# hungdinhxuan/real-time-deepfake-speech-detection

Hardware: AMD Instinct MI355X
Metric: utterances/sec (4 s @ 16 kHz) (higher is better)
Workload: dtype fp16

## Files before the change

### real-time-deepfake-speech-detection_amd/csrc/afx_conformer.hip

```cpp
#include "afx_common.h"
#include "afx_kernels.h"

namespace afx {

__global__ void conf_tokens_kernel(const float* __restrict__ ll, const float* __restrict__ cls, float bn_scale,
                                   float bn_shift, int T, int E, float* __restrict__ out, int raw) {
  const int b = blockIdx.y;
  const long n = (long)(T + 1) * E;
  for (long i = (long)blockIdx.x * blockDim.x + threadIdx.x; i < n; i += (long)gridDim.x * blockDim.x) {
    const int row = (int)(i / E), c = (int)(i % E);
    float v;
    if (row == 0)
      v = cls[c];
    else if (raw)
      v = ll[((long)b * T + row - 1) * E + c];
    else
      v = selu(fmaf(ll[((long)b * T + row - 1) * E + c], bn_scale, bn_shift));
    out[(long)b * n + i] = v;
  }
}
const char* launch_conf_tokens(const float* ll, const float* cls, float bn_scale, float bn_shift, int B, int T,
                               int E, float* out, hipStream_t s, bool raw) {
  hipLaunchKernelGGL(conf_tokens_kernel, dim3(16, B), dim3(256), 0, s, ll, cls, bn_scale, bn_shift, T, E, out, raw ? 1 : 0);
  hipError_t e = hipGetLastError();
// ... 129 lines not shown
  if ((ldq % 4) || (ldkv % 4) || (ldo % 4)) return "conf_attn: row strides must be multiples of 4";
  hipError_t e = hipSuccess;
#define AFX_CA(DHv)                                                                                             \
  AFX_DISPATCH_HT(dtype, e = launch_conf_attn_t<DHv, HT, true>(q, ldq, kv, ldkv, rel, max_pos, B, N, H, out_h, ldo, s, lens, len_add))
  if (!rel) {
    if (dh != 64 || dtype != DT_FP32) return "conf_attn: the no-relative-term form is the fp32 trunk attention (dh 64)";
    e = launch_conf_attn_t<64, F32T, false>(q, ldq, kv, ldkv, nullptr, 0, B, N, H, out_h, ldo, s, lens, len_add);
  }
  else if (dh == 36) { AFX_CA(36); }
  else if (dh == 32) { AFX_CA(32); }
  else if (dh == 64) { AFX_CA(64); }
  else return "conf_attn: supported head dims are 32, 36 (emb 144 / 4 heads) and 64";
#undef AFX_CA
  return e == hipSuccess ? nullptr : hipGetErrorString(e);
}

constexpr int CA_KEYS = 224, CA_VT_STRIDE = 232, CA_RS = 228, CA_NKT = 14, CA_KS = 7;

template <class HT, int DH, int NW>
__global__ __launch_bounds__(64 * NW) void conf_attn_mfma_kernel(const float* __restrict__ q, long ldq,
                                                             const float* __restrict__ kv, long ldkv,
                                                             const typename HT::T* __restrict__ rel_h, int max_pos,
                                                             int N, int H, typename HT::T* __restrict__ out, long ldo,
                                                             const int* __restrict__ lens, int len_add) {
  typedef typename HT::T Tt;
  typedef typename HT::V8 V8;
  typedef typename HT::V4 V4;
  const int Nrow = N;
  if (lens) N = lens[blockIdx.y] + len_add;
  constexpr int DT = (DH + 15) / 16;
  static_assert(DH % 4 == 0 && DH <= 64, "head dim");
  extern __shared__ __attribute__((aligned(16))) float sm_f[];
  char* sm = (char*)sm_f;
  char* k_lds = sm;
  Tt* vt_lds = (Tt*)(sm + CA_KEYS * 128);
  float* r_lds = (float*)(sm + CA_KEYS * 128 + 16 * DT * CA_VT_STRIDE * 2);
  constexpr int NT = 64 * NW;

  const int h = blockIdx.x, b = blockIdx.y;
  const int tid = threadIdx.x, lane = tid & 63, wave = tid >> 6;
  const int inner = H * DH;
  for (int i = tid; i < (CA_KEYS * 128 + 16 * DT * CA_VT_STRIDE * 2) / 16; i += NT) ((u32x4*)sm)[i] = u32x4{0u, 0u, 0u, 0u};
  __syncthreads();
  {
    constexpr int IT = (209 * (DH / 4) + NT - 1) / NT;
    f32x4 kreg[IT], vreg[IT];
#pragma unroll
// ... 6 lines not shown
        vreg[it] = *(const f32x4*)(row + inner);
      }
    }
#pragma unroll
    for (int it = 0; it < IT; ++it) {
      const int idx = tid + it * NT;
      if (idx < N * (DH / 4)) {
        const int key = idx / (DH / 4), q4 = idx % (DH / 4);
        V4 kh;
#pragma unroll
        for (int i = 0; i < 4; ++i) kh[i] = (Tt)kreg[it][i];
        const int c = q4 >> 1;
        *(V4*)(k_lds + key * 128 + ((c ^ ((key >> 1) & 7)) * 16) + (q4 & 1) * 8) = kh;
#pragma unroll
        for (int i = 0; i < 4; ++i) vt_lds[(q4 * 4 + i) * CA_VT_STRIDE + key] = (Tt)vreg[it][i];
      }
    }
  }
  __syncthreads();

  const int ql = lane & 15, g = lane >> 4;
  const float scale = 1.0f / sqrtf((float)DH);
  float* rw = r_lds + wave * 16 * CA_RS;
  const int nqt = (N + 15) >> 4;
  for (int qt = wave; qt < nqt; qt += NW) {
    const int q0 = qt * 16;
    int qrow = q0 + ql;
    qrow = qrow < N ? qrow : N - 1;
    V8 qf[2];
    {
      const float* qp = q + ((long)b * Nrow + qrow) * ldq + h * DH;
#pragma unroll
      for (int ks = 0; ks < 2; ++ks)
#pragma unroll
        for (int half = 0; half < 2; ++half) {
          const int d = ks * 32 + g * 8 + half * 4;
          f32x4 t = f32x4{0.f, 0.f, 0.f, 0.f};
          if (d < DH) t = *(const f32x4*)(qp + d);
#pragma unroll
          for (int i = 0; i < 4; ++i) qf[ks][half * 4 + i] = (Tt)(t[i] * scale);
        }
    }
    auto read_e = [&](int rp, V8 (&ef)[2][2]) {
#pragma unroll
      for (int u = 0; u < 2; ++u) {
        int er = q0 + (rp + u) * 16 + ql - (N - 1);
        er = er < -max_pos ? -max_pos : (er > max_pos ? max_pos : er);
// ... 102 lines not shown
#pragma unroll
      for (int nt = 0; nt < DT; ++nt) o[nt] = HT::mfma(vf[nt], pf, o[nt]);
      __builtin_amdgcn_sched_barrier(0);
    }
    const int qi = q0 + ql;
    if (qi < N) {
#pragma unroll
      for (int nt = 0; nt < DT; ++nt) {
        const int d = nt * 16 + g * 4;
        if (d < DH) {
          V4 hv;
#pragma unroll
          for (int c = 0; c < 4; ++c) hv[c] = (Tt)(o[nt][c] * rinv);
          *(V4*)(out + ((long)b * Nrow + qi) * ldo + h * DH + d) = hv;
        }
      }
    }
  }
}

template <int DH, int NW>
__global__ __launch_bounds__(64 * NW) void conf_attn_split_kernel(const float* __restrict__ q, long ldq, const float* __restrict__ kv, long ldkv,
                                                                  const float* __restrict__ rel64, int max_pos, int N, int H,
                                                                  float* __restrict__ out, long ldo, const int* __restrict__ lens, int len_add) {
  typedef _Float16 Tt;
  typedef f16x8 V8;
  typedef f16x4 V4;
  const int Nrow = N;
  if (lens) N = lens[blockIdx.y] + len_add;
  constexpr int DT = (DH + 15) / 16;
  static_assert(DH % 4 == 0 && DH <= 64, "head dim");
  extern __shared__ __attribute__((aligned(16))) float sm_f[];
  char* sm = (char*)sm_f;
  constexpr int KB = CA_KEYS * 128, VB = 16 * DT * CA_VT_STRIDE * 2;
  char* k_lds[2] = {sm, sm + KB};
  Tt* vt_lds[2] = {(Tt*)(sm + 2 * KB), (Tt*)(sm + 2 * KB + VB)};
  float* r_lds = (float*)(sm + 2 * KB + 2 * VB);
  constexpr int NT = 64 * NW;
  const int h = blockIdx.x, b = blockIdx.y;
  const int tid = threadIdx.x, lane = tid & 63, wave = tid >> 6;
  const int inner = H * DH;
  auto split4 = [](const f32x4& a, V4& hi, V4& lo) {
#pragma unroll
    for (int i = 0; i < 4; ++i) {
      hi[i] = (Tt)a[i];
      lo[i] = (Tt)(a[i] - (float)hi[i]);
    }
// ... 27 lines not shown
      const int idx = tid + it * NT;
      if (idx < N * (DH / 4)) {
        const int key = idx / (DH / 4), q4 = idx % (DH / 4);
        V4 kh, kl, vh, vl;
        split4(kreg[it], kh, kl);
        split4(vreg[it], vh, vl);
        const int c = q4 >> 1;
        const int off = key * 128 + ((c ^ ((key >> 1) & 7)) * 16) + (q4 & 1) * 8;
        *(V4*)(k_lds[0] + off) = kh;
        *(V4*)(k_lds[1] + off) = kl;
#pragma unroll
        for (int i = 0; i < 4; ++i) {
          vt_lds[0][(q4 * 4 + i) * CA_VT_STRIDE + key] = vh[i];
          vt_lds[1][(q4 * 4 + i) * CA_VT_STRIDE + key] = vl[i];
        }
      }
    }
  }
  __syncthreads();

  const int ql = lane & 15, g = lane >> 4;
  const float scale = 1.0f / sqrtf((float)DH);
  float* rw = r_lds + wave * 16 * CA_RS;
  const int nqt = (N + 15) >> 4;
  for (int qt = wave; qt < nqt; qt += NW) {
    const int q0 = qt * 16;
    int qrow = q0 + ql;
    qrow = qrow < N ? qrow : N - 1;
    V8 qh[2], qlo[2];
    {
      const float* qp = q + ((long)b * Nrow + qrow) * ldq + h * DH;
#pragma unroll
      for (int ks = 0; ks < 2; ++ks) {
        f32x4 t[2];
#pragma unroll
        for (int half = 0; half < 2; ++half) {
          const int d = ks * 32 + g * 8 + half * 4;
          t[half] = f32x4{0.f, 0.f, 0.f, 0.f};
          if (d < DH) t[half] = *(const f32x4*)(qp + d);
        }
        split8(t[0], t[1], qh[ks], qlo[ks]);
      }
    }
    auto read_e = [&](int rp, f32x4 (&ef)[2][2][2]) {
#pragma unroll
      for (int u = 0; u < 2; ++u) {
        int er = q0 + (rp + u) * 16 + ql - (N - 1);
// ... 113 lines not shown
        o[nt] = FP16::mfma(vf[nt][1], ph, o[nt]);
        o[nt] = FP16::mfma(vf[nt][0], pl, o[nt]);
        o[nt] = FP16::mfma(vf[nt][0], ph, o[nt]);
      }
      __builtin_amdgcn_sched_barrier(0);
    }
    const int qi = q0 + ql;
    if (qi < N) {
#pragma unroll
      for (int nt = 0; nt < DT; ++nt) {
        const int d = nt * 16 + g * 4;
        if (d < DH) *(f32x4*)(out + ((long)b * Nrow + qi) * ldo + h * DH + d) = o[nt] * rinv;
      }
#ifdef SHAW_DBG
      if (g == 0) {
        out[((long)b * Nrow + qi) * ldo + h * DH + 0] = mx;
        out[((long)b * Nrow + qi) * ldo + h * DH + 1] = sum;
      }
#endif
    }
  }
}
const char* launch_conf_attn_split(const float* q, long ldq, const float* kv, long ldkv, const float* rel64, int max_pos, int B, int N,
                                   int H, int dh, float* out, long ldo, hipStream_t s, const int* lens, int len_add) {
  if (dh != 36) return "conf_attn_split: built for head dim 36 (emb 144 / 4 heads)";
  if (N <= 0 || N + 15 > CA_KEYS || B <= 0 || B > 65535) return "conf_attn_split: 1..209 tokens";
  if ((ldq % 4) || (ldkv % 4) || (ldo % 4)) return "conf_attn_split: row strides must be multiples of 4";
  constexpr int DT = 3, NW = 4;
  const int lds = 2 * CA_KEYS * 128 + 2 * 16 * DT * CA_VT_STRIDE * 2 + NW * 16 * CA_RS * 4;
  static LdsLimit lim;
  hipError_t e = lim.ensure((const void*)conf_attn_split_kernel<36, NW>, lds);
  if (e == hipSuccess) {
    hipLaunchKernelGGL((conf_attn_split_kernel<36, NW>), dim3(H, B), dim3(64 * NW), lds, s, q, ldq, kv, ldkv, rel64, max_pos, N, H, out, ldo, lens, len_add);
    e = hipGetLastError();
  }
  return e == hipSuccess ? nullptr : hipGetErrorString(e);
}

constexpr int CAL_KB = 128, CAL_VT_STRIDE = 136, CAL_RS = 148, CAL_NKT = 8, CAL_KS = 4, CAL_RT = 9;

template <class HT, int DH>
__global__ __launch_bounds__(256, 2) void conf_attn_mfma_long_kernel(const float* __restrict__ q, long ldq,
                                                                  const float* __restrict__ kv, long ldkv,
                                                                  const typename HT::T* __restrict__ rel_h, int max_pos,
                                                                  int N, int H, typename HT::T* __restrict__ out, long ldo,
                                                                  const int* __restrict__ lens, int len_add) {
  typedef typename HT::T Tt;
  typedef typename HT::V8 V8;
  typedef typename HT::V4 V4;
  const int Nrow = N;
  if (lens) N = lens[blockIdx.y] + len_add;
  constexpr int DT = (DH + 15) / 16;
  static_assert(DH % 4 == 0 && DH <= 64, "head dim");
  extern __shared__ __attribute__((aligned(16))) float sm_f[];
  char* sm = (char*)sm_f;
  char* k_lds = sm;
  Tt* vt_lds = (Tt*)(sm + CAL_KB * 128);
  float* r_lds = (float*)(sm + CAL_KB * 128 + 16 * DT * CAL_VT_STRIDE * 2);
  const int h = blockIdx.x, b = blockIdx.y;
  const int tid = threadIdx.x, lane = tid & 63, wave = tid >> 6;
  const int inner = H * DH;
  const int ql = lane & 15, g = lane >> 4;
  const int q0 = blockIdx.z * 64 + wave * 16;
  const float scale = 1.0f / sqrtf((float)DH);
  float* rw = r_lds + wave * 16 * CAL_RS;
  for (int i = tid; i < (CAL_KB * 128 + 16 * DT * CAL_VT_STRIDE * 2) / 16; i += 256) ((u32x4*)sm)[i] = u32x4{0u, 0u, 0u, 0u};
  V8 qf[2];
  {
    const int qrow = q0 + ql < N ? q0 + ql : N - 1;
// ... 26 lines not shown
        if (idx < nk * (DH / 4)) {
          const int key = idx / (DH / 4), q4 = idx % (DH / 4);
          const float* row = kv + ((long)b * Nrow + j0 + key) * ldkv + h * DH + q4 * 4;
          kreg[it] = *(const f32x4*)row;
          vreg[it] = *(const f32x4*)(row + inner);
        }
      }
#pragma unroll
      for (int it = 0; it < IT; ++it) {
        const int idx = tid + it * 256;
        if (idx < nk * (DH / 4)) {
          const int key = idx / (DH / 4), q4 = idx % (DH / 4);
          V4 kh;
#pragma unroll
          for (int i = 0; i < 4; ++i) kh[i] = (Tt)kreg[it][i];
          const int c = q4 >> 1;
          *(V4*)(k_lds + key * 128 + ((c ^ ((key >> 1) & 7)) * 16) + (q4 & 1) * 8) = kh;
#pragma unroll
          for (int i = 0; i < 4; ++i) vt_lds[(q4 * 4 + i) * CAL_VT_STRIDE + key] = (Tt)vreg[it][i];
        }
      }
    }
    __syncthreads();
    if (q0 >= N) continue;

    const int base = q0 - j0 - (CAL_KB - 1);
#pragma unroll
    for (int rp = 0; rp < CAL_RT; ++rp) {
      int er = base + rp * 16 + ql;
      er = er < -max_pos ? -max_pos : (er > max_pos ? max_pos : er);
      const Tt* ep = rel_h + (long)(er + max_pos) * 64 + g * 8;
      const V8 e0 = *(const V8*)ep, e1 = *(const V8*)(ep + 32);
      f32x4 r2 = f32x4{0.f, 0.f, 0.f, 0.f};
      r2 = HT::mfma(e0, qf[0], r2);
      r2 = HT::mfma(e1, qf[1], r2);
      *(f32x4*)(rw + ql * CAL_RS + rp * 16 + g * 4) = r2;
    }
    f32x4 s[CAL_NKT];
#pragma unroll
    for (int kp = 0; kp < CAL_NKT; kp += 2) {
      V8 kf[2][2];
#pragma unroll
      for (int u = 0; u < 2; ++u) {
        const int krow = (kp + u) * 16 + ql;
        const int sw = (krow >> 1) & 7;
#pragma unroll
        for (int ks = 0; ks < 2; ++ks) kf[u][ks] = *(const V8*)(k_lds + krow * 128 + (((ks * 4 + g) ^ sw) * 16));
// ... 35 lines not shown
      V8 pf;
#pragma unroll
      for (int c = 0; c < 4; ++c) {
        pf[c] = (Tt)s[2 * s2][c];
        pf[4 + c] = (Tt)s[2 * s2 + 1][c];
      }
      V8 vf[DT];
#pragma unroll
      for (int nt = 0; nt < DT; ++nt) {
        const Tt* vr = vt_lds + (nt * 16 + ql) * CAL_VT_STRIDE + s2 * 32 + g * 4;
        const V4 lo = *(const V4*)vr;
        const V4 hi = *(const V4*)(vr + 16);
#pragma unroll
        for (int c = 0; c < 4; ++c) {
          vf[nt][c] = lo[c];
          vf[nt][4 + c] = hi[c];
        }
      }
#pragma unroll
      for (int nt = 0; nt < DT; ++nt) o[nt] = HT::mfma(vf[nt], pf, o[nt]);
    }
  }
  const int qi = q0 + ql;
  if (qi < N) {
    const float rinv = 1.0f / l;
#pragma unroll
    for (int nt = 0; nt < DT; ++nt) {
      const int d = nt * 16 + g * 4;
      if (d < DH) {
        V4 hv;
#pragma unroll
        for (int c = 0; c < 4; ++c) hv[c] = (Tt)(o[nt][c] * rinv);
        *(V4*)(out + ((long)b * Nrow + qi) * ldo + h * DH + d) = hv;
      }
    }
  }
}

static int g_conf_attn_force_long = 0;
void conf_attn_mfma_set_force_long(int v) { g_conf_attn_force_long = v != 0; }
static int g_conf_attn_waves = 7;
void conf_attn_mfma_set_waves(int v) { g_conf_attn_waves = v == 4 ? 4 : 7; }

const char* launch_conf_attn_mfma(const float* q, long ldq, const float* kv, long ldkv, const void* rel_h, int max_pos,
                                  int B, int N, int H, int dh, void* out_h, long ldo, int dtype, hipStream_t s,
                                  const int* lens, int len_add) {
  if (dh != 36) return "conf_attn_mfma: built for head dim 36 (emb 144 / 4 heads)";
  if (N <= 0 || B <= 0 || B > 65535) return "conf_attn_mfma: bad shape";
  if (dtype == DT_FP32) return "conf_attn_mfma: half-precision operands only";
  if ((ldq % 4) || (ldkv % 4) || (ldo % 4)) return "conf_attn_mfma: row strides must be multiples of 4";
  constexpr int DT = 3;
  if (N + 15 > CA_KEYS || g_conf_attn_force_long) {
    const int ldsl = CAL_KB * 128 + 16 * DT * CAL_VT_STRIDE * 2 + 4 * 16 * CAL_RS * 4;
    hipError_t el = hipSuccess;
    static LdsLimit liml[2];
    dim3 grid(H, B, (N + 63) / 64);
    if (dtype == DT_BF16) {
      el = liml[0].ensure((const void*)conf_attn_mfma_long_kernel<BF16, 36>, ldsl);
      if (el == hipSuccess)
        hipLaunchKernelGGL((conf_attn_mfma_long_kernel<BF16, 36>), grid, dim3(256), ldsl, s, q, ldq, kv, ldkv, (const __bf16*)rel_h,
                           max_pos, N, H, (__bf16*)out_h, ldo, lens, len_add);
    } else {
      el = liml[1].ensure((const void*)conf_attn_mfma_long_kernel<FP16, 36>, ldsl);
      if (el == hipSuccess)
        hipLaunchKernelGGL((conf_attn_mfma_long_kernel<FP16, 36>), grid, dim3(256), ldsl, s, q, ldq, kv, ldkv, (const _Float16*)rel_h,
                           max_pos, N, H, (_Float16*)out_h, ldo, lens, len_add);
    }
    if (el == hipSuccess) el = hipGetLastError();
    return el == hipSuccess ? nullptr : hipGetErrorString(el);
  }
  const int nw = N > 64 && g_conf_attn_waves != 4 ? 7 : 4;
  const int lds = CA_KEYS * 128 + 16 * DT * CA_VT_STRIDE * 2 + nw * 16 * CA_RS * 4;
  hipError_t e = hipSuccess;
  static LdsLimit lim[4];
#define AFX_CAM(HTv, NWv, slot, Tv)                                                                                      \
  do {                                                                                                                   \
    e = lim[slot].ensure((const void*)conf_attn_mfma_kernel<HTv, 36, NWv>, lds);                                         \
    if (e == hipSuccess)                                                                                                 \
      hipLaunchKernelGGL((conf_attn_mfma_kernel<HTv, 36, NWv>), dim3(H, B), dim3(64 * NWv), lds, s, q, ldq, kv, ldkv,    \
                         (const Tv*)rel_h, max_pos, N, H, (Tv*)out_h, ldo, lens, len_add);                               \
  } while (0)
  if (dtype == DT_BF16) {
    if (nw == 7) AFX_CAM(BF16, 7, 0, __bf16); else AFX_CAM(BF16, 4, 1, __bf16);
  } else {
    if (nw == 7) AFX_CAM(FP16, 7, 2, _Float16); else AFX_CAM(FP16, 4, 3, _Float16);
  }
#undef AFX_CAM
  if (e == hipSuccess) e = hipGetLastError();
  return e == hipSuccess ? nullptr : hipGetErrorString(e);
}

template <class HT>
__global__ __launch_bounds__(256) void conf_dwconv_kernel(const float* __restrict__ x, long ldx,
                                                          const float* __restrict__ w, const float* __restrict__ bias,
                                                          const float* __restrict__ bn_scale,
                                                          const float* __restrict__ bn_shift, int N, int NC, int C, int k,
                                                          typename HT::T* __restrict__ out, long ldo,
                                                          const int* __restrict__ lens, int len_add) {
  typedef typename HT::T Tt;
  const int Nrow = N;
  if (lens) N = lens[blockIdx.y] + len_add;
  constexpr bool EXACT = sizeof(Tt) == 4;
  constexpr int KMAX = 31, TB = 8;
  extern __shared__ __attribute__((aligned(16))) float sm_f[];
  float* sm = sm_f;
  const int c0 = blockIdx.x * 32, b = blockIdx.y, tid = threadIdx.x;
  const int pl = k / 2;
  const int f0 = blockIdx.z * NC, nc = min(NC, N - f0);
  const int rows = nc + KMAX - 1 + TB;
  float* us = sm;
  const int cl = tid & 31, tl = tid >> 5;
  const int c = c0 + cl;
  const bool cok = c < C;
  for (int r = tl; r < rows; r += 8) {
    const int t = f0 + r - pl;
    float u = 0.f;
    if (cok && t >= 0 && t < N) {
      const float* row = x + ((long)b * Nrow + t) * ldx;
      u = row[c] * (EXACT ? sigmoid_acc(row[C + c]) : sigmoid_fast(row[C + c]));
    }
    us[r * 32 + cl] = u;
  }
  float wr[KMAX];
#pragma unroll
  for (int j = 0; j < KMAX; ++j) wr[j] = (cok && j < k) ? w[(long)c * k + j] : 0.f;
  const float bi = cok ? bias[c] : 0.f, sc = cok ? bn_scale[c] : 0.f, sh = cok ? bn_shift[c] : 0.f;
  __syncthreads();
  const int per = (nc + 7) / 8;
  const int t_end = min(nc, (tl + 1) * per);
  for (int t0 = tl * per; t0 < t_end; t0 += TB) {
    float win[TB + KMAX - 1];
#pragma unroll
    for (int i = 0; i < TB + KMAX - 1; ++i) win[i] = us[(t0 + i) * 32 + cl];
    float acc[TB];
#pragma unroll
    for (int u = 0; u < TB; ++u) acc[u] = bi;
#pragma unroll
    for (int j = 0; j < KMAX; ++j)
#pragma unroll
      for (int u = 0; u < TB; ++u) acc[u] = fmaf(wr[j], win[u + j], acc[u]);
    if (cok) {
#pragma unroll
      for (int u = 0; u < TB; ++u) {
        const float y = fmaf(acc[u], sc, sh);
        if (t0 + u < t_end) out[((long)b * Nrow + f0 + t0 + u) * ldo + c] = (Tt)(EXACT ? swish(y) : swish_fast(y));
      }
    }
  }
}

const char* launch_conf_dwconv(const float* x, long ldx, const float* w, const float* bias, const float* bn_scale,
                               const float* bn_shift, int B, int N, int C, int k, void* out_h, long ldo, int dtype,
                               hipStream_t s, const int* lens, int len_add) {
  if (k > 31) return "conf_dwconv: depthwise kernels up to 31 taps";
  if (N <= 0 || B <= 0 || B > 65535) return "conf_dwconv: bad shape";
  const int NC = N < 1024 ? N : 1024;
  const int lds = (NC + 31 - 1 + 8) * 32 * (int)sizeof(float);
  dim3 grid((C + 31) / 32, B, (N + NC - 1) / NC);
  hipError_t e = hipSuccess;
  static LdsLimit lim[3];
  if (dtype < 0 || dtype > 2) return "conf_dwconv: unknown dtype";
  AFX_DISPATCH_HT(dtype, {
    e = lim[dtype].ensure((const void*)conf_dwconv_kernel<HT>, lds);
    if (e == hipSuccess)
      hipLaunchKernelGGL(conf_dwconv_kernel<HT>, grid, dim3(256), lds, s, x, ldx, w, bias, bn_scale, bn_shift, N, NC, C, k,
                         (HT::T*)out_h, ldo, lens, len_add);
  });
  if (e == hipSuccess) e = hipGetLastError();
  return e == hipSuccess ? nullptr : hipGetErrorString(e);
}

__global__ void small_linear_kernel(const float* __restrict__ x, long row_stride, int rows, int K,
                                    const float* __restrict__ w, const float* __restrict__ b, int N,
                                    float* __restrict__ out, int* __restrict__ nonfinite) {
  const int lane = threadIdx.x & 63;
  const int r = blockIdx.x * (blockDim.x >> 6) + (threadIdx.x >> 6);
  if (r >= rows) return;
  const float* xr = x + (long)r * row_stride;
  for (int n = 0; n < N; ++n) {
    float a = 0.f;
    for (int kk = lane; kk < K; kk += 64) a = fmaf(xr[kk], w[(long)n * K + kk], a);
    a = wave_sum(a);
    if (lane == 0) {
      a += b ? b[n] : 0.f;
      out[(long)r * N + n] = a;
      if (nonfinite && !(fabsf(a) <= 3.0e38f)) atomicAdd(nonfinite, 1);
    }
  }
}
// ... 10 lines not shown
```

### real-time-deepfake-speech-detection_amd/csrc/afx_conformer_fused.hip

```cpp
#include "afx_common.h"
#include "afx_kernels.h"

#ifndef CHAIN_DBG
#define CHAIN_DBG 0
#endif

namespace afx {

namespace {

constexpr int ET = 9;
constexpr int EK = 5;
constexpr int HT6 = 6;
constexpr int RING = 4, BUFSZ = 32 * 1024, DUMP = RING * BUFSZ;
constexpr int PARAMS = DUMP + 1024;
template <int N>
__device__ __forceinline__ void chain_wait_vmcnt() {
  static_assert(N >= 0 && N < 64, "vmcnt is a 6-bit counter");
  asm volatile("s_waitcnt vmcnt(%0)" ::"n"(N) : "memory");
}

struct ChunkDesc {
  const void* W;
  int ldw, n0, k0, nt, ks;
// ... 287 lines not shown
          v[r] = swish_of(v[r]);
        }
        hf[t] = pack_pair(u, v);
      }
      mm<ET, 3, true>(hf, o);
    }
    descale<ET>(o, CS_FF2);
#pragma unroll
    for (int j = 0; j < ET; ++j) {
      const f32x4 bb = *(const f32x4*)(prm + CP_FF_B2 + j * 16 + kq * 4);
      x[j] += 0.5f * (o[j] + bb);
    }
  }
};

}

template <class HT, int STAGE, bool S3, int NWAVE>
__global__ __launch_bounds__(64 * NWAVE) void conf_chain_kernel(ConfChainArgs p) {
  typedef Chain<HT, STAGE, S3, NWAVE> C;
  typedef typename C::AF AF;
  extern __shared__ __attribute__((aligned(16))) char smem[];
  C c(p, smem);
  const long row = ((long)blockIdx.x * NWAVE + c.wave) * 16 + c.r16;
  const bool ok = row < p.M;
  const long rc = ok ? row : p.M - 1;

  f32x4 x[ET];
#pragma unroll
  for (int j = 0; j < ET; ++j) x[j] = *(const f32x4*)(p.x_in + rc * p.E + j * 16 + c.kq * 4);
  AF ain[ET];
  if constexpr (STAGE != 0) {
#pragma unroll
    for (int t = 0; t < (STAGE == 1 ? EK : ET); ++t) ain[t] = c.load_frag(p.in_h, rc, p.ld_in_h, t * 32 + c.kb);
  }
#pragma unroll
  for (int j = 0; j < ET; ++j) asm volatile("" : "+v"(x[j]));
  if constexpr (STAGE != 0) {
#pragma unroll
    for (int t = 0; t < (STAGE == 1 ? EK : ET); ++t) {
      asm volatile("" : "+v"(ain[t].h));
      if constexpr (S3) asm volatile("" : "+v"(ain[t].l));
    }
  }
  c.prologue();

  if constexpr (STAGE == 0) {
    c.feed_forward(x);
    if (ok) {
// ... 71 lines not shown
  static LdsLimit lim;
  if (hipError_t e = lim.ensure((const void*)conf_chain_kernel<HT, STAGE, S3, NWAVE>, lds); e != hipSuccess) return e;
  hipLaunchKernelGGL((conf_chain_kernel<HT, STAGE, S3, NWAVE>), dim3((unsigned)((p.M + 16 * NWAVE - 1) / (16 * NWAVE))), dim3(64 * NWAVE), lds, s, p);
  return hipGetLastError();
}
template <class HT, bool S3, int NWAVE>
static hipError_t launch_conf_chain_s(const ConfChainArgs& p, int stage, hipStream_t s) {
  return stage == 0 ? launch_conf_chain_t<HT, 0, S3, NWAVE>(p, s) : stage == 1 ? launch_conf_chain_t<HT, 1, S3, NWAVE>(p, s) : launch_conf_chain_t<HT, 2, S3, NWAVE>(p, s);
}

static int g_chain_waves = 0;
void conf_chain_set_waves(int v) { g_chain_waves = v == 4 || v == 8 ? v : 0; }
int conf_chain_waves_of(int M, int obj) {
  if (g_chain_waves) return g_chain_waves;
  if (!dispatch_cu(obj, CU_CHAIN_WAVES)) return 4;
  const long w4 = (M + 63) / 64, w8 = (M + 127) / 128;
  return w8 * 309 < w4 * 273 ? 8 : 4;
}

const char* launch_conf_chain(const ConfChainArgs& p, int stage, int dtype, hipStream_t s) {
  if (p.E != 16 * ET || p.Ep < 32 * EK || p.FFp != 4 * 16 * ET) return "conf_chain: the fused Conformer chains are built for emb 144 / ff 576";
  if (dtype == DT_FP32) return "conf_chain: half-precision operands only";
  if (p.M <= 0 || stage < 0 || stage > 2) return "conf_chain: bad arguments";
  const bool w8 = conf_chain_waves_of(p.M, dispatch_objective(p.objective)) == 8;
  hipError_t e;
  if (dtype == DT_FP16X3)
    e = w8 ? launch_conf_chain_s<FP16, true, 8>(p, stage, s) : launch_conf_chain_s<FP16, true, 4>(p, stage, s);
  else if (dtype == DT_BF16)
    e = w8 ? launch_conf_chain_s<BF16, false, 8>(p, stage, s) : launch_conf_chain_s<BF16, false, 4>(p, stage, s);
  else
    e = w8 ? launch_conf_chain_s<FP16, false, 8>(p, stage, s) : launch_conf_chain_s<FP16, false, 4>(p, stage, s);
  return e == hipSuccess ? nullptr : hipGetErrorString(e);
}

}
```

### real-time-deepfake-speech-detection_amd/csrc/afx_engine.hip

```cpp
#include <hip/hip_runtime.h>

#include <algorithm>
#include <cmath>
#include <cstdarg>
#include <cstdio>
#include <cstring>
#include <string>
#include <unordered_map>
#include <unordered_set>
#include <vector>

#include "../../include/afx.h"
#include "afx_common.h"
#include "afx_kernels.h"
#include "afx_aasist.h"
#include "afx_entry.h"

using namespace afx;

static thread_local char g_err[512] = "";
int afx::fail(const char* fmt, ...) {
  va_list ap;
  va_start(ap, fmt);
  vsnprintf(g_err, sizeof g_err, fmt, ap);
// ... 66 lines not shown
struct ConfBlock {
  void *ff1_w1, *ff1_w2, *ff2_w1, *ff2_w2, *wqkv, *wout, *pw1, *pw2;
  float *bn_scale, *bn_shift;
  void* rel_h;
  float* chain_prm[3];
};

struct Profiler;

struct afx_engine {
  afx_config cfg;
  bool s3 = false;
  Profiler* prof = nullptr;
  int dt;
  size_t hsz;
  std::vector<void*> allocs;
  std::unordered_map<std::string, FT> f;
  std::unordered_set<std::string> loaded;
  bool finalized = false;
  bool taps_on = false;
  int posconv_sliding = 1;
  int conf_attn_mfma = 1;
  int fuse_conformer = 1;
  int fuse_conv_ln = 1;
  int gemm_small_deep = 1;
  int concurrent = 0;
  int last_objective = 0;
  std::unordered_map<std::string, TapRec> taps;
  int* nonfinite = nullptr;
  std::unordered_map<const float*, float> ln_scale;

  void* convw[7] = {nullptr};
  void* conv0pack = nullptr;
  void* projw = nullptr;
  void* posw = nullptr;
  float* pos_norm = nullptr;
  std::vector<void*> wqkv, wo, w1, w2;
  std::vector<float*> bqkv;
  int E = 0, Ep = 0, heads = 0, dh = 0, inner = 0, FF = 0, FFp = 0, C2 = 0, C2p = 0, ck = 0, nblk = 0;
  void* conf_ll = nullptr;
  float conf_bn_scale = 1.f, conf_bn_shift = 0.f;
  std::vector<ConfBlock> blk;
  AasistWeights aw;

  void* walloc(size_t rows, size_t k) { return dalloc(rows * k * hsz + (s3 ? rows * 4 : 0)); }
  float* wscale(const void* w, size_t rows, size_t k) const { return s3 ? (float*)((char*)w + rows * k * 4) : nullptr; }
// ... 1018 lines not shown
  HIP_OK(hipMemsetAsync(w.ao, 0, (size_t)M * Ep * hs, s));
  if (!fused) {
    HIP_OK(hipMemsetAsync(w.hc, 0, (size_t)M * Ep * hs, s));
    HIP_OK(hipMemsetAsync(w.u, 0, (size_t)M * e->C2p * hs, s));
    if (e->FFp != e->FF) HIP_OK(hipMemsetAsync(w.hid, 0, (size_t)M * e->FFp * hs, s));
  }
  for (int b = 0; fused && b < e->nblk; ++b) {
    const std::string P = "conformer.encoder_blocks." + std::to_string(b) + ".";
    ConfBlock& K = e->blk[b];
    ConfChainArgs c;
    memset(&c, 0, sizeof c);
    c.M = M; c.E = E; c.Ep = Ep; c.FFp = e->FFp; c.objective = cx.objective;
    c.x_in = w.xc; c.x_out = w.xc;
    auto ff = [&](void* w1, void* w2) { c.ff_w1 = w1; c.ff_w2 = w2; };
    const double ff_fl = 2.0 * M * E * e->FF * 2;
    ff(K.ff1_w1, K.ff1_w2);
    c.params = K.chain_prm[0];
    c.w_a = K.wqkv; c.ld_w_a = Ep;
    c.out2 = w.qkv32; c.ld_out2 = 3 * e->inner;
    KOK(cx.timed(PC_CONF_CHAIN, ff_fl + 2.0 * M * E * 3 * e->inner, [&] { return launch_conf_chain(c, 0, chain_dt, s); }));
    const std::string bp = "b" + std::to_string(b) + ".";
    TAP(bp + "xa", w.xc, (size_t)M * E, false, E);
    TAP(bp + "qkv", w.qkv32, (size_t)M * 3 * e->inner, false, 3 * e->inner);
    KOK(cx.timed(PC_CONF_ATTN, 6.0 * B * e->heads * (double)N * N * e->dh, [&] {
      if (e->conf_attn_mfma && dt != DT_FP32 && e->dh == 36)
        return launch_conf_attn_mfma(w.qkv32, 3 * e->inner, w.qkv32 + e->inner, 3 * e->inner, K.rel_h, 512, B, N, e->heads,
                                     e->dh, w.ao, Ep, dt, s, w.lens, 1);
      if (e->conf_attn_mfma && e->s3 && e->dh == 36 && N <= 209)
        return launch_conf_attn_split(w.qkv32, 3 * e->inner, w.qkv32 + e->inner, 3 * e->inner, (const float*)K.rel_h, 512, B, N,
                                      e->heads, e->dh, (float*)w.ao, Ep, s, w.lens, 1);
      return launch_conf_attn(w.qkv32, 3 * e->inner, w.qkv32 + e->inner, 3 * e->inner,
                              e->F(P + "attn.fn.rel_pos_emb.weight"), 512, B, N, e->heads, e->dh, w.ao, Ep, dt, s, w.lens, 1);
    }));
    TAP(bp + "ao", w.ao, (size_t)M * Ep, true, Ep);
    c.in_h = w.ao; c.ld_in_h = Ep;
    c.params = K.chain_prm[1];
    c.w_a = K.wout;
    c.w_b = K.pw1;
    c.out2 = w.glu32; c.ld_out2 = 2 * e->C2;
    KOK(cx.timed(PC_CONF_CHAIN, 2.0 * M * E * (e->inner + 2 * e->C2), [&] { return launch_conf_chain(c, 1, chain_dt, s); }));
    TAP(bp + "xb", w.xc, (size_t)M * E, false, E);
    TAP(bp + "glu", w.glu32, (size_t)M * 2 * e->C2, false, 2 * e->C2);
    KOK(cx.timed(PC_CONF_DWCONV, 2.0 * B * N * e->C2 * e->ck, [&] {
      return launch_conf_dwconv(w.glu32, 2 * e->C2, e->F(P + "conv.net.4.conv.weight"),
                                e->F(P + "conv.net.4.conv.bias"), K.bn_scale, K.bn_shift, B, N, e->C2, e->ck, w.u,
                                e->C2p, dt, s, w.lens, 1);
    }));
    TAP(bp + "u", w.u, (size_t)M * e->C2p, true, e->C2p);
    c.in_h = w.u; c.ld_in_h = e->C2p;
    c.params = K.chain_prm[2];
    c.w_a = K.pw2; c.ld_w_a = e->C2p;
    ff(K.ff2_w1, K.ff2_w2);
    c.w_b = nullptr; c.out2 = nullptr;
    KOK(cx.timed(PC_CONF_CHAIN, ff_fl + 2.0 * M * e->C2 * E, [&] { return launch_conf_chain(c, 2, chain_dt, s); }));
    if (e->taps_on) {
      const std::string nm = "block" + std::to_string(b);
      if (tap(cx, nm.c_str(), w.xc, (size_t)M * E, false)) return 1;
    }
  }
  for (int b = 0; !fused && b < e->nblk; ++b) {
    const std::string P = "conformer.encoder_blocks." + std::to_string(b) + ".";
    ConfBlock& K = e->blk[b];
    const std::string bp = "b" + std::to_string(b) + ".";
    auto norm_to_h = [&](const char* nm) -> const char* {
      RowNormArgs n = plain_norm(w.xc, E, M, E, e->F(P + nm + ".weight"), e->F(P + nm + ".bias"));
      n.out_h = w.hc; n.ldo_h = Ep;
      return cx.rownorm(n, dt);
    };
    auto feed_forward = [&](const char* ff, void* w1, void* w2) -> int {
      KOK(norm_to_h((std::string(ff) + ".fn.norm").c_str()));
      TAP(bp + ff + ".hc", w.hc, (size_t)M * Ep, true, Ep);
      GemmArgs a = plain_gemm(w.hc, Ep, w1, Ep, M, e->FF, Ep);
      a.k_algo = E;
      a.bias = e->F(P + ff + ".fn.fn.net.0.bias"); a.act = ACT_SWISH;
      a.out_h = w.hid; a.ldo_h = e->FFp;
      KOK(cx.gemm(a, dt, 1));
      TAP(bp + ff + ".hid", w.hid, (size_t)M * e->FFp, true, e->FFp);
// ... 1228 lines not shown
    gemm_set_deep(value);
    return 0;
  }
  if (!strcmp(key, "gemm_nodma")) {
    if (!gemm_set_nodma(value)) return fail("afx_debug_set: gemm_nodma exists only in the attribution build (make attr, AFX_LIB=.../libafx_attr.so)");
    return 0;
  }
  if (!strcmp(key, "gemm_a_nt")) {
    gemm_set_a_nt(value);
    return 0;
  }
  if (!strcmp(key, "conv0_mfma")) {
    conv0_set_mfma(value);
    return 0;
  }

  return fail("afx_debug_set: unknown key '%s'", key);
}
extern "C" int afx_engine_set(afx_handle h, const char* key, int value) {
  if (!h || !key) return fail("afx_engine_set: null argument");
  if (!strcmp(key, "posconv_sliding")) h->posconv_sliding = value != 0;
  else if (!strcmp(key, "conf_attn_mfma")) h->conf_attn_mfma = value != 0;
  else if (!strcmp(key, "fuse_conformer")) h->fuse_conformer = value != 0;
  else if (!strcmp(key, "fuse_conv_ln")) h->fuse_conv_ln = value != 0;
  else if (!strcmp(key, "gemm_small_deep")) h->gemm_small_deep = value != 0;
  else if (!strcmp(key, "concurrent")) h->concurrent = value != 0;
  else return fail("afx_engine_set: unknown key '%s'", key);
  return 0;
}
extern "C" int afx_engine_get(afx_handle h, const char* key, int* value) {
  if (!h || !key || !value) return fail("afx_engine_get: null argument");
  if (!strcmp(key, "concurrent")) *value = h->concurrent;
  else if (!strcmp(key, "objective")) *value = h->last_objective;
  else return fail("afx_engine_get: unknown key '%s'", key);
  return 0;
}
extern "C" int afx_gemm_plan(int M, int N, int K, int rpb, int kchunk, int groups, int flags, int objective, int* out) {
  if (!out || M <= 0 || N <= 0 || K <= 0 || groups <= 0) return fail("afx_gemm_plan: bad arguments");
  GemmArgs g = plain_gemm(nullptr, K, nullptr, K, M, N, K);
  if (rpb > 0) g.rpb = rpb;
  if (kchunk > 0) g.kchunk = kchunk;
  if (flags & 1) g.ln_gamma = g.ln_beta = g.bias = (const float*)out;
  if (flags & 2) { g.k1 = K; g.K = 2 * K; g.kchunk = 2 * g.kchunk; }
  if (flags & 4) g.act = ACT_SWISH;
  if (flags & 8) g.no_deep = 1;
  const int obj = objective < 0 ? dispatch_objective(OBJ_MAKESPAN) : (objective ? OBJ_CU_TIME : OBJ_MAKESPAN);
// ... 43 lines not shown
```

### real-time-deepfake-speech-detection_amd/csrc/afx_kernels.h

```cpp
#pragma once
#include <hip/hip_runtime.h>
#include <stdint.h>

namespace afx {

enum DType { DT_BF16 = 0, DT_FP16 = 1, DT_FP32 = 2, DT_FP16X3 = 3 };
inline size_t dtype_size(int dt) { return dt == DT_FP32 || dt == DT_FP16X3 ? 4 : 2; }
constexpr float kS3ScaleBounded = 16.f;
constexpr float kS3ScaleFree = 1.f;
__host__ __device__ inline long s3_pair_index(long k) { return ((k >> 5) << 6) + (k & 31); }

struct GemmArgs {
  const void* A;
  const void* W;
  int M, N, K;
  int k_algo;
  int rpb;
  long a_batch, a_row;
  int kchunk;
  long kchunk_stride;
  long ldw;
  long g_a, g_w;
  int g_n;
  const float* bias;
// ... 118 lines not shown
const char* launch_posconv(const PosConvArgs& p, int dtype, hipStream_t s);

const char* launch_mhsa(const void* qkv, void* out, int B, int T, int H, int dtype, hipStream_t s, const int* lens = nullptr);
void mhsa_set_vtr(int v);

const char* launch_mhsa_split(const float* qkv, float* out, int B, int T, int H, hipStream_t s, const int* lens = nullptr,
                              bool out_pairs = false, float out_scale = 1.f);
struct MhsaRingForm {
  int form;
  int q_tile;
  const int* cnt;
  const int* tab;
};
const char* launch_mhsa_ring(const void* ring, void* out, int S, int H, const MhsaRingForm& f, int dtype, hipStream_t s);
const char* launch_mhsa_ring_split(const float* ring, float* out, int S, int H, const MhsaRingForm& f, hipStream_t s,
                                   bool out_pairs = false, float out_scale = 1.f);

const char* launch_conf_tokens(const float* ll, const float* cls, float bn_scale, float bn_shift, int B, int T,
                               int E, float* out, hipStream_t s, bool raw = false);
const char* launch_conf_attn(const float* q, long ldq, const float* kv, long ldkv, const float* rel, int max_pos,
                             int B, int N, int H, int dh, void* out_h, long ldo, int dtype, hipStream_t s,
                             const int* lens = nullptr, int len_add = 0);
const char* launch_conf_attn_split(const float* q, long ldq, const float* kv, long ldkv, const float* rel64, int max_pos, int B, int N,
                                   int H, int dh, float* out, long ldo, hipStream_t s, const int* lens = nullptr, int len_add = 0);
const char* launch_conf_attn_mfma(const float* q, long ldq, const float* kv, long ldkv, const void* rel_h, int max_pos,
                                  int B, int N, int H, int dh, void* out_h, long ldo, int dtype, hipStream_t s,
                                  const int* lens = nullptr, int len_add = 0);
const char* launch_conf_dwconv(const float* x, long ldx, const float* w , const float* bias,
                               const float* bn_scale, const float* bn_shift, int B, int N, int C, int k,
                               void* out_h, long ldo, int dtype, hipStream_t s, const int* lens = nullptr, int len_add = 0);
enum ChainParamOffsets { CP_FF_G = 0, CP_FF_B = 144, CP_FF_B1 = 288, CP_FF_B2 = 864, CP_LN2_G = 1008, CP_LN2_B = 1152,
                         CP_BA = 1296, CP_BB = 1440 };
constexpr int kChainParamFloats = 2048;
constexpr int kChainScaleFloats = 2048;
enum ChainScaleOffsets { CS_FF1 = 0, CS_FF2 = 576, CS_A = 720, CS_B = 1152 };
static_assert(CS_B + 576 <= kChainScaleFloats, "scale block");
struct ConfChainArgs {
  int M, E, Ep, FFp;
  const float* x_in;
  float* x_out;
  const float* params;
  const void *ff_w1, *ff_w2;
  const void* w_a;
  int ld_w_a;
  int objective;
  const void* w_b;
  const void* in_h;
  long ld_in_h;
  float* out2;
  long ld_out2;
};
const char* launch_conf_chain(const ConfChainArgs& p, int stage, int dtype, hipStream_t s);
void conf_chain_set_waves(int v);
int conf_chain_waves_of(int M, int objective);
const char* launch_small_linear(const float* x, long row_stride, int rows, int K, const float* w, const float* b,
                                int N, float* out, hipStream_t s, int* nonfinite = nullptr);

}
```

Baseline: 13970.

## Restrict last Conformer block to the CLS token's dependency cone

In the final Conformer block only the CLS token's output is needed, so attention query rows, the GLU chain, and the depthwise conv are limited to the rows that can reach token 0. Attention computes queries only for the first reach_right+1 tokens. The chain operates on a grouped row map of nq rows per batch, and the conv and second chain compute only one output row per utterance. This removes most of the last block's compute but leaves the non-CLS rows of the final activations stale, which is only valid if downstream reads just the CLS token. Taps disable it.

```diff
diff --git a/real-time-deepfake-speech-detection_amd/csrc/afx_conformer.hip b/real-time-deepfake-speech-detection_amd/csrc/afx_conformer.hip
--- a/real-time-deepfake-speech-detection_amd/csrc/afx_conformer.hip
+++ b/real-time-deepfake-speech-detection_amd/csrc/afx_conformer.hip
@@ -1,3 +1,5 @@
+#include <climits>
+
 #include "afx_common.h"
 #include "afx_kernels.h"
 
@@ -175,7 +177,7 @@
                                                              const float* __restrict__ kv, long ldkv,
                                                              const typename HT::T* __restrict__ rel_h, int max_pos,
                                                              int N, int H, typename HT::T* __restrict__ out, long ldo,
-                                                             const int* __restrict__ lens, int len_add) {
+                                                             const int* __restrict__ lens, int len_add, int nq) {
   typedef typename HT::T Tt;
   typedef typename HT::V8 V8;
   typedef typename HT::V4 V4;
@@ -228,7 +230,7 @@
   const int ql = lane & 15, g = lane >> 4;
   const float scale = 1.0f / sqrtf((float)DH);
   float* rw = r_lds + wave * 16 * CA_RS;
-  const int nqt = (N + 15) >> 4;
+  const int nqt = (min(N, nq) + 15) >> 4;
   for (int qt = wave; qt < nqt; qt += NW) {
     const int q0 = qt * 16;
     int qrow = q0 + ql;
@@ -377,7 +379,8 @@
 template <int DH, int NW>
 __global__ __launch_bounds__(64 * NW) void conf_attn_split_kernel(const float* __restrict__ q, long ldq, const float* __restrict__ kv, long ldkv,
                                                                   const float* __restrict__ rel64, int max_pos, int N, int H,
-                                                                  float* __restrict__ out, long ldo, const int* __restrict__ lens, int len_add) {
+                                                                  float* __restrict__ out, long ldo, const int* __restrict__ lens, int len_add,
+                                                                  int nq) {
   typedef _Float16 Tt;
   typedef f16x8 V8;
   typedef f16x4 V4;
@@ -451,7 +454,7 @@
   const int ql = lane & 15, g = lane >> 4;
   const float scale = 1.0f / sqrtf((float)DH);
   float* rw = r_lds + wave * 16 * CA_RS;
-  const int nqt = (N + 15) >> 4;
+  const int nqt = (min(N, nq) + 15) >> 4;
   for (int qt = wave; qt < nqt; qt += NW) {
     const int q0 = qt * 16;
     int qrow = q0 + ql;
@@ -611,8 +614,9 @@
   }
 }
 const char* launch_conf_attn_split(const float* q, long ldq, const float* kv, long ldkv, const float* rel64, int max_pos, int B, int N,
-                                   int H, int dh, float* out, long ldo, hipStream_t s, const int* lens, int len_add) {
+                                   int H, int dh, float* out, long ldo, hipStream_t s, const int* lens, int len_add, int nq) {
   if (dh != 36) return "conf_attn_split: built for head dim 36 (emb 144 / 4 heads)";
+  if (nq <= 0) nq = INT_MAX;
   if (N <= 0 || N + 15 > CA_KEYS || B <= 0 || B > 65535) return "conf_attn_split: 1..209 tokens";
   if ((ldq % 4) || (ldkv % 4) || (ldo % 4)) return "conf_attn_split: row strides must be multiples of 4";
   constexpr int DT = 3, NW = 4;
@@ -620,7 +624,7 @@
   static LdsLimit lim;
   hipError_t e = lim.ensure((const void*)conf_attn_split_kernel<36, NW>, lds);
   if (e == hipSuccess) {
-    hipLaunchKernelGGL((conf_attn_split_kernel<36, NW>), dim3(H, B), dim3(64 * NW), lds, s, q, ldq, kv, ldkv, rel64, max_pos, N, H, out, ldo, lens, len_add);
+    hipLaunchKernelGGL((conf_attn_split_kernel<36, NW>), dim3(H, B), dim3(64 * NW), lds, s, q, ldq, kv, ldkv, rel64, max_pos, N, H, out, ldo, lens, len_add, nq);
     e = hipGetLastError();
   }
   return e == hipSuccess ? nullptr : hipGetErrorString(e);
@@ -633,7 +637,7 @@
                                                                   const float* __restrict__ kv, long ldkv,
                                                                   const typename HT::T* __restrict__ rel_h, int max_pos,
                                                                   int N, int H, typename HT::T* __restrict__ out, long ldo,
-                                                                  const int* __restrict__ lens, int len_add) {
+                                                                  const int* __restrict__ lens, int len_add, int nq) {
   typedef typename HT::T Tt;
   typedef typename HT::V8 V8;
   typedef typename HT::V4 V4;
@@ -706,7 +710,7 @@
       }
     }
     __syncthreads();
-    if (q0 >= N) continue;
+    if (q0 >= min(N, nq)) continue;
 
     const int base = q0 - j0 - (CAL_KB - 1);
 #pragma unroll
@@ -788,7 +792,7 @@
     }
   }
   const int qi = q0 + ql;
-  if (qi < N) {
+  if (qi < N && q0 < nq) {
     const float rinv = 1.0f / l;
 #pragma unroll
     for (int nt = 0; nt < DT; ++nt) {
@@ -810,8 +814,10 @@
 
 const char* launch_conf_attn_mfma(const float* q, long ldq, const float* kv, long ldkv, const void* rel_h, int max_pos,
                                   int B, int N, int H, int dh, void* out_h, long ldo, int dtype, hipStream_t s,
-                                  const int* lens, int len_add) {
+                                  const int* lens, int len_add, int nq) {
   if (dh != 36) return "conf_attn_mfma: built for head dim 36 (emb 144 / 4 heads)";
+  if (nq <= 0) nq = INT_MAX;
+  const int NQ = N < nq ? N : nq;
   if (N <= 0 || B <= 0 || B > 65535) return "conf_attn_mfma: bad shape";
   if (dtype == DT_FP32) return "conf_attn_mfma: half-precision operands only";
   if ((ldq % 4) || (ldkv % 4) || (ldo % 4)) return "conf_attn_mfma: row strides must be multiples of 4";
@@ -820,22 +826,22 @@
     const int ldsl = CAL_KB * 128 + 16 * DT * CAL_VT_STRIDE * 2 + 4 * 16 * CAL_RS * 4;
     hipError_t el = hipSuccess;
     static LdsLimit liml[2];
-    dim3 grid(H, B, (N + 63) / 64);
+    dim3 grid(H, B, (NQ + 63) / 64);
     if (dtype == DT_BF16) {
       el = liml[0].ensure((const void*)conf_attn_mfma_long_kernel<BF16, 36>, ldsl);
       if (el == hipSuccess)
         hipLaunchKernelGGL((conf_attn_mfma_long_kernel<BF16, 36>), grid, dim3(256), ldsl, s, q, ldq, kv, ldkv, (const __bf16*)rel_h,
-                           max_pos, N, H, (__bf16*)out_h, ldo, lens, len_add);
+                           max_pos, N, H, (__bf16*)out_h, ldo, lens, len_add, nq);
     } else {
       el = liml[1].ensure((const void*)conf_attn_mfma_long_kernel<FP16, 36>, ldsl);
       if (el == hipSuccess)
         hipLaunchKernelGGL((conf_attn_mfma_long_kernel<FP16, 36>), grid, dim3(256), ldsl, s, q, ldq, kv, ldkv, (const _Float16*)rel_h,
-                           max_pos, N, H, (_Float16*)out_h, ldo, lens, len_add);
+                           max_pos, N, H, (_Float16*)out_h, ldo, lens, len_add, nq);
     }
     if (el == hipSuccess) el = hipGetLastError();
     return el == hipSuccess ? nullptr : hipGetErrorString(el);
   }
-  const int nw = N > 64 && g_conf_attn_waves != 4 ? 7 : 4;
+  const int nw = NQ > 64 && g_conf_attn_waves != 4 ? 7 : 4;
   const int lds = CA_KEYS * 128 + 16 * DT * CA_VT_STRIDE * 2 + nw * 16 * CA_RS * 4;
   hipError_t e = hipSuccess;
   static LdsLimit lim[4];
@@ -844,7 +850,7 @@
     e = lim[slot].ensure((const void*)conf_attn_mfma_kernel<HTv, 36, NWv>, lds);                                         \
     if (e == hipSuccess)                                                                                                 \
       hipLaunchKernelGGL((conf_attn_mfma_kernel<HTv, 36, NWv>), dim3(H, B), dim3(64 * NWv), lds, s, q, ldq, kv, ldkv,    \
-                         (const Tv*)rel_h, max_pos, N, H, (Tv*)out_h, ldo, lens, len_add);                               \
+                         (const Tv*)rel_h, max_pos, N, H, (Tv*)out_h, ldo, lens, len_add, nq);                           \
   } while (0)
   if (dtype == DT_BF16) {
     if (nw == 7) AFX_CAM(BF16, 7, 0, __bf16); else AFX_CAM(BF16, 4, 1, __bf16);
@@ -862,17 +868,18 @@
                                                           const float* __restrict__ bn_scale,
                                                           const float* __restrict__ bn_shift, int N, int NC, int C, int k,
                                                           typename HT::T* __restrict__ out, long ldo,
-                                                          const int* __restrict__ lens, int len_add) {
+                                                          const int* __restrict__ lens, int len_add, int nf) {
   typedef typename HT::T Tt;
   const int Nrow = N;
   if (lens) N = lens[blockIdx.y] + len_add;
+  const int Nout = min(N, nf);
   constexpr bool EXACT = sizeof(Tt) == 4;
   constexpr int KMAX = 31, TB = 8;
   extern __shared__ __attribute__((aligned(16))) float sm_f[];
   float* sm = sm_f;
   const int c0 = blockIdx.x * 32, b = blockIdx.y, tid = threadIdx.x;
-  const int pl = k / 2;
-  const int f0 = blockIdx.z * NC, nc = min(NC, N - f0);
+  const int pl = conf_dwconv_pad_left(k);
+  const int f0 = blockIdx.z * NC, nc = min(NC, Nout - f0);
   const int rows = nc + KMAX - 1 + TB;
   float* us = sm;
   const int cl = tid & 31, tl = tid >> 5;
@@ -917,12 +924,14 @@
 
 const char* launch_conf_dwconv(const float* x, long ldx, const float* w, const float* bias, const float* bn_scale,
                                const float* bn_shift, int B, int N, int C, int k, void* out_h, long ldo, int dtype,
-                               hipStream_t s, const int* lens, int len_add) {
+                               hipStream_t s, const int* lens, int len_add, int nf) {
   if (k > 31) return "conf_dwconv: depthwise kernels up to 31 taps";
   if (N <= 0 || B <= 0 || B > 65535) return "conf_dwconv: bad shape";
-  const int NC = N < 1024 ? N : 1024;
+  if (nf <= 0) nf = INT_MAX;
+  const int Nout = N < nf ? N : nf;
+  const int NC = Nout < 1024 ? Nout : 1024;
   const int lds = (NC + 31 - 1 + 8) * 32 * (int)sizeof(float);
-  dim3 grid((C + 31) / 32, B, (N + NC - 1) / NC);
+  dim3 grid((C + 31) / 32, B, (Nout + NC - 1) / NC);
   hipError_t e = hipSuccess;
   static LdsLimit lim[3];
   if (dtype < 0 || dtype > 2) return "conf_dwconv: unknown dtype";
@@ -930,7 +939,7 @@
     e = lim[dtype].ensure((const void*)conf_dwconv_kernel<HT>, lds);
     if (e == hipSuccess)
       hipLaunchKernelGGL(conf_dwconv_kernel<HT>, grid, dim3(256), lds, s, x, ldx, w, bias, bn_scale, bn_shift, N, NC, C, k,
-                         (HT::T*)out_h, ldo, lens, len_add);
+                         (HT::T*)out_h, ldo, lens, len_add, nf);
   });
   if (e == hipSuccess) e = hipGetLastError();
   return e == hipSuccess ? nullptr : hipGetErrorString(e);
diff --git a/real-time-deepfake-speech-detection_amd/csrc/afx_conformer_fused.hip b/real-time-deepfake-speech-detection_amd/csrc/afx_conformer_fused.hip
--- a/real-time-deepfake-speech-detection_amd/csrc/afx_conformer_fused.hip
+++ b/real-time-deepfake-speech-detection_amd/csrc/afx_conformer_fused.hip
@@ -333,9 +333,11 @@
   typedef typename C::AF AF;
   extern __shared__ __attribute__((aligned(16))) char smem[];
   C c(p, smem);
-  const long row = ((long)blockIdx.x * NWAVE + c.wave) * 16 + c.r16;
-  const bool ok = row < p.M;
-  const long rc = ok ? row : p.M - 1;
+  const long lrow = ((long)blockIdx.x * NWAVE + c.wave) * 16 + c.r16;
+  const bool ok = lrow < p.M;
+  const int lrc = ok ? (int)lrow : p.M - 1;
+  const long rc = p.grp_rows > 0 ? (long)(lrc / p.grp_rows) * p.grp_stride + lrc % p.grp_rows : lrc;
+  const long row = rc;
 
   f32x4 x[ET];
 #pragma unroll
@@ -453,6 +455,7 @@
   if (p.E != 16 * ET || p.Ep < 32 * EK || p.FFp != 4 * 16 * ET) return "conf_chain: the fused Conformer chains are built for emb 144 / ff 576";
   if (dtype == DT_FP32) return "conf_chain: half-precision operands only";
   if (p.M <= 0 || stage < 0 || stage > 2) return "conf_chain: bad arguments";
+  if (p.grp_rows < 0 || (p.grp_rows > 0 && p.grp_stride < p.grp_rows)) return "conf_chain: bad row map (groups must not overlap)";
   const bool w8 = conf_chain_waves_of(p.M, dispatch_objective(p.objective)) == 8;
   hipError_t e;
   if (dtype == DT_FP16X3)
diff --git a/real-time-deepfake-speech-detection_amd/csrc/afx_engine.hip b/real-time-deepfake-speech-detection_amd/csrc/afx_engine.hip
--- a/real-time-deepfake-speech-detection_amd/csrc/afx_engine.hip
+++ b/real-time-deepfake-speech-detection_amd/csrc/afx_engine.hip
@@ -112,6 +112,7 @@
   int posconv_sliding = 1;
   int conf_attn_mfma = 1;
   int fuse_conformer = 1;
+  int conf_cone = 1;
   int fuse_conv_ln = 1;
   int gemm_small_deep = 1;
   int concurrent = 0;
@@ -1176,13 +1177,17 @@
     const std::string bp = "b" + std::to_string(b) + ".";
     TAP(bp + "xa", w.xc, (size_t)M * E, false, E);
     TAP(bp + "qkv", w.qkv32, (size_t)M * 3 * e->inner, false, 3 * e->inner);
-    KOK(cx.timed(PC_CONF_ATTN, 6.0 * B * e->heads * (double)N * N * e->dh, [&] {
+    const bool cone = e->conf_cone && !e->taps_on && b == e->nblk - 1;
+    const int cone_g = std::min(conf_dwconv_reach_right(e->ck) + 1, N);
+    const int nq = cone ? cone_g : N;
+    const bool attn_mc = e->conf_attn_mfma && e->dh == 36 && (dt != DT_FP32 || (e->s3 && N <= 209));
+    KOK(cx.timed(PC_CONF_ATTN, 6.0 * B * e->heads * (double)(attn_mc ? nq : N) * N * e->dh, [&] {
       if (e->conf_attn_mfma && dt != DT_FP32 && e->dh == 36)
         return launch_conf_attn_mfma(w.qkv32, 3 * e->inner, w.qkv32 + e->inner, 3 * e->inner, K.rel_h, 512, B, N, e->heads,
-                                     e->dh, w.ao, Ep, dt, s, w.lens, 1);
+                                     e->dh, w.ao, Ep, dt, s, w.lens, 1, cone ? nq : 0);
       if (e->conf_attn_mfma && e->s3 && e->dh == 36 && N <= 209)
         return launch_conf_attn_split(w.qkv32, 3 * e->inner, w.qkv32 + e->inner, 3 * e->inner, (const float*)K.rel_h, 512, B, N,
-                                      e->heads, e->dh, (float*)w.ao, Ep, s, w.lens, 1);
+                                      e->heads, e->dh, (float*)w.ao, Ep, s, w.lens, 1, cone ? nq : 0);
       return launch_conf_attn(w.qkv32, 3 * e->inner, w.qkv32 + e->inner, 3 * e->inner,
                               e->F(P + "attn.fn.rel_pos_emb.weight"), 512, B, N, e->heads, e->dh, w.ao, Ep, dt, s, w.lens, 1);
     }));
@@ -1192,13 +1197,14 @@
     c.w_a = K.wout;
     c.w_b = K.pw1;
     c.out2 = w.glu32; c.ld_out2 = 2 * e->C2;
-    KOK(cx.timed(PC_CONF_CHAIN, 2.0 * M * E * (e->inner + 2 * e->C2), [&] { return launch_conf_chain(c, 1, chain_dt, s); }));
+    if (cone) { c.M = B * nq; c.grp_rows = nq; c.grp_stride = N; }
+    KOK(cx.timed(PC_CONF_CHAIN, 2.0 * c.M * E * (e->inner + 2 * e->C2), [&] { return launch_conf_chain(c, 1, chain_dt, s); }));
     TAP(bp + "xb", w.xc, (size_t)M * E, false, E);
     TAP(bp + "glu", w.glu32, (size_t)M * 2 * e->C2, false, 2 * e->C2);
-    KOK(cx.timed(PC_CONF_DWCONV, 2.0 * B * N * e->C2 * e->ck, [&] {
+    KOK(cx.timed(PC_CONF_DWCONV, 2.0 * B * (cone ? 1 : N) * e->C2 * e->ck, [&] {
       return launch_conf_dwconv(w.glu32, 2 * e->C2, e->F(P + "conv.net.4.conv.weight"),
                                 e->F(P + "conv.net.4.conv.bias"), K.bn_scale, K.bn_shift, B, N, e->C2, e->ck, w.u,
-                                e->C2p, dt, s, w.lens, 1);
+                                e->C2p, dt, s, w.lens, 1, cone ? 1 : 0);
     }));
     TAP(bp + "u", w.u, (size_t)M * e->C2p, true, e->C2p);
     c.in_h = w.u; c.ld_in_h = e->C2p;
@@ -1206,7 +1212,8 @@
     c.w_a = K.pw2; c.ld_w_a = e->C2p;
     ff(K.ff2_w1, K.ff2_w2);
     c.w_b = nullptr; c.out2 = nullptr;
-    KOK(cx.timed(PC_CONF_CHAIN, ff_fl + 2.0 * M * e->C2 * E, [&] { return launch_conf_chain(c, 2, chain_dt, s); }));
+    if (cone) { c.M = B; c.grp_rows = 1; c.grp_stride = N; }
+    KOK(cx.timed(PC_CONF_CHAIN, 2.0 * c.M * E * e->FF * 2 + 2.0 * c.M * e->C2 * E, [&] { return launch_conf_chain(c, 2, chain_dt, s); }));
     if (e->taps_on) {
       const std::string nm = "block" + std::to_string(b);
       if (tap(cx, nm.c_str(), w.xc, (size_t)M * E, false)) return 1;
@@ -2481,6 +2488,7 @@
   if (!strcmp(key, "posconv_sliding")) h->posconv_sliding = value != 0;
   else if (!strcmp(key, "conf_attn_mfma")) h->conf_attn_mfma = value != 0;
   else if (!strcmp(key, "fuse_conformer")) h->fuse_conformer = value != 0;
+  else if (!strcmp(key, "conf_cone")) h->conf_cone = value != 0;
   else if (!strcmp(key, "fuse_conv_ln")) h->fuse_conv_ln = value != 0;
   else if (!strcmp(key, "gemm_small_deep")) h->gemm_small_deep = value != 0;
   else if (!strcmp(key, "concurrent")) h->concurrent = value != 0;
diff --git a/real-time-deepfake-speech-detection_amd/csrc/afx_kernels.h b/real-time-deepfake-speech-detection_amd/csrc/afx_kernels.h
--- a/real-time-deepfake-speech-detection_amd/csrc/afx_kernels.h
+++ b/real-time-deepfake-speech-detection_amd/csrc/afx_kernels.h
@@ -164,13 +164,17 @@
                              int B, int N, int H, int dh, void* out_h, long ldo, int dtype, hipStream_t s,
                              const int* lens = nullptr, int len_add = 0);
 const char* launch_conf_attn_split(const float* q, long ldq, const float* kv, long ldkv, const float* rel64, int max_pos, int B, int N,
-                                   int H, int dh, float* out, long ldo, hipStream_t s, const int* lens = nullptr, int len_add = 0);
+                                   int H, int dh, float* out, long ldo, hipStream_t s, const int* lens = nullptr, int len_add = 0,
+                                   int nq = 0);
 const char* launch_conf_attn_mfma(const float* q, long ldq, const float* kv, long ldkv, const void* rel_h, int max_pos,
                                   int B, int N, int H, int dh, void* out_h, long ldo, int dtype, hipStream_t s,
-                                  const int* lens = nullptr, int len_add = 0);
+                                  const int* lens = nullptr, int len_add = 0, int nq = 0);
 const char* launch_conf_dwconv(const float* x, long ldx, const float* w , const float* bias,
                                const float* bn_scale, const float* bn_shift, int B, int N, int C, int k,
-                               void* out_h, long ldo, int dtype, hipStream_t s, const int* lens = nullptr, int len_add = 0);
+                               void* out_h, long ldo, int dtype, hipStream_t s, const int* lens = nullptr, int len_add = 0,
+                               int nf = 0);
+constexpr int conf_dwconv_pad_left(int k) { return k / 2; }
+constexpr int conf_dwconv_reach_right(int k) { return k - 1 - k / 2; }
 enum ChainParamOffsets { CP_FF_G = 0, CP_FF_B = 144, CP_FF_B1 = 288, CP_FF_B2 = 864, CP_LN2_G = 1008, CP_LN2_B = 1152,
                          CP_BA = 1296, CP_BB = 1440 };
 constexpr int kChainParamFloats = 2048;
@@ -179,6 +183,7 @@
 static_assert(CS_B + 576 <= kChainScaleFloats, "scale block");
 struct ConfChainArgs {
   int M, E, Ep, FFp;
+  int grp_rows, grp_stride;
   const float* x_in;
   float* x_out;
   const float* params;
```

Measured after the change: 13990 (median of 3 runs). No clear change (+0.2%).
